# apache/cloudberry

Hardware: AMD Instinct MI355X
Metric: tpch_q3_rows_per_sec (higher is better)
Workload: dtype f64; 1 GPU; tpch_q3_sf100; lineitem_rows=599977225, parallelism=mpp1, lineitem_key_format=none, groups=12779481

## Files before the change

### cloudberry_amd/__init__.py

```python
import ctypes
import os

import numpy as np

_ROOT = os.path.dirname(os.path.dirname(os.path.abspath(__file__)))
_SO = os.path.join(_ROOT, "cloudberry_amd", "libgpuexec.so")

TPCH_CUSTOMER, TPCH_ORDERS, TPCH_LINEITEM = 0, 1, 2
TPCH_LINEITEM_NUMERIC = 3
TPCH_LINEITEM_RLEKEY = 4
TPCH_LINEITEM_Q1 = 5
CUTOFF_19950315 = -1753

_STATUS = {0: "GX_OK", 1: "GX_ERR_HIP", 2: "GX_ERR_RCCL", 3: "GX_ERR_INVALID",
           4: "GX_ERR_CHECKSUM", 5: "GX_ERR_OOM", 6: "GX_ERR_NOGPU", 7: "GX_ERR_STATE"}


class GxError(RuntimeError):
    def __init__(self, status, detail=""):
        self.status = status
        super().__init__(f"{_STATUS.get(status, status)}: {detail}")


class _Group(ctypes.Structure):
# ... 204 lines not shown
                                    ctypes.POINTER(ctypes.c_int64),
                                    ctypes.POINTER(_GbStats)]
    lib.gx_test_gb_partial.argtypes = [ctypes.c_void_p, ctypes.c_void_p,
                                       ctypes.c_int, ctypes.c_int, ctypes.c_int,
                                       ctypes.c_void_p, ctypes.c_void_p,
                                       ctypes.c_int64,
                                       ctypes.POINTER(ctypes.c_int64)]
    lib.gx_test_gb_combine.argtypes = [ctypes.c_void_p, ctypes.c_void_p,
                                       ctypes.c_int64,
                                       ctypes.POINTER(ctypes.POINTER(_KvGroup)),
                                       ctypes.POINTER(ctypes.c_int64)]
    lib.gx_partition_multi.argtypes = [ctypes.c_void_p, ctypes.c_void_p,
                                       ctypes.c_void_p, ctypes.c_void_p,
                                       ctypes.c_int32, ctypes.c_int64,
                                       ctypes.c_int32, ctypes.c_void_p]
    lib.gx_q3_prepare.argtypes = [ctypes.c_void_p] * 4 + [ctypes.c_int32,
                                  ctypes.POINTER(ctypes.c_void_p)]
    lib.gx_q3_prepare_desc.argtypes = [ctypes.c_void_p, ctypes.POINTER(_Q3Desc),
                                       ctypes.POINTER(ctypes.c_void_p)]
    lib.gx_q3_set_numeric.argtypes = [ctypes.c_void_p, ctypes.c_int]
    lib.gx_q3_run.argtypes = [ctypes.c_void_p]
    lib.gx_q3_stats_get.argtypes = [ctypes.c_void_p, ctypes.POINTER(_Stats)]
    lib.gx_q3_dim_mode.argtypes = [ctypes.c_void_p, ctypes.POINTER(ctypes.c_int)]
    lib.gx_q3_result.argtypes = [ctypes.c_void_p, ctypes.POINTER(ctypes.POINTER(_Group)),
                                 ctypes.POINTER(ctypes.c_int64)]
    lib.gx_q3_topn.argtypes = [ctypes.c_void_p, ctypes.c_int, ctypes.c_void_p,
                               ctypes.POINTER(ctypes.c_int64)]
    lib.gx_q3_free.argtypes = [ctypes.c_void_p]
    lib.gx_free.argtypes = [ctypes.c_void_p]
    lib.gx_test_motion1.argtypes = [ctypes.c_void_p, ctypes.c_void_p, ctypes.c_int32,
                                    ctypes.c_int, ctypes.c_void_p, ctypes.c_void_p,
                                    ctypes.c_int64, ctypes.POINTER(ctypes.c_int64)]
    lib.gx_test_qual.argtypes = [ctypes.c_void_p, ctypes.c_void_p, ctypes.c_void_p,
                                 ctypes.c_int64, ctypes.c_int, ctypes.c_void_p,
                                 ctypes.c_void_p, ctypes.c_int64,
                                 ctypes.POINTER(ctypes.c_int64)]
    lib.gx_test_q3_from_qual.argtypes = [ctypes.c_void_p, ctypes.c_void_p,
                                         ctypes.c_int64, ctypes.c_void_p,
                                         ctypes.c_int32,
                                         ctypes.POINTER(ctypes.POINTER(_Group)),
                                         ctypes.POINTER(ctypes.c_int64)]
    lib.gx_test_m1.argtypes = [ctypes.c_void_p, ctypes.c_void_p,
                               ctypes.POINTER(_Filter), ctypes.c_int,
                               ctypes.c_int, ctypes.c_void_p, ctypes.c_uint64,
                               ctypes.c_void_p, ctypes.c_void_p,
                               ctypes.c_int64, ctypes.POINTER(ctypes.c_int64)]
# ... 91 lines not shown
    rc = lib().gx_selftest_motion_layout(
        c.ctypes.data, n, seg, scnt.ctypes.data, soff.ctypes.data,
        rcnt.ctypes.data, roff.ctypes.data, 0, 0, 0, 1, 300, None)
    if rc != 0:
        raise ValueError(f"gx_selftest_motion_layout: bad arguments ({rc})")
    return scnt, soff, rcnt, roff


def motion_table_layout(qual, kmin, kmax, nsegs, tf_pct=300):
    lay = _TblLayout()
    rc = lib().gx_selftest_motion_layout(None, 0, 0, None, None, None, None,
                                         qual, kmin, kmax, nsegs, tf_pct,
                                         ctypes.byref(lay))
    if rc != 0:
        raise ValueError(f"gx_selftest_motion_layout: bad arguments ({rc})")
    return _layout_dict(lay)


def unmatched_bound(nrows, lmin, lmax):
    return int(lib().gx_selftest_unmatched_bound(
        int(nrows), int(lmin) & (2**64 - 1), int(lmax) & (2**64 - 1)))


def gb_lds_groups(naggs):
    return int(lib().gx_gb_lds_groups(naggs))


def gb_sort(keys, key_null):
    keys = np.ascontiguousarray(keys, np.int64)
    key_null = np.ascontiguousarray(key_null, np.uint8)
    assert keys.ndim == 2 and keys.shape == key_null.shape
    n, nkeys = keys.shape
    perm = np.zeros(n, np.int64)
    rc = lib().gx_selftest_gb_sort(keys.ctypes.data, key_null.ctypes.data, n,
                                   nkeys, perm.ctypes.data)
    if rc != 0:
        raise ValueError(f"gx_selftest_gb_sort: bad arguments ({rc})")
    return perm


def _gb_desc(table, keys, aggs, quals, max_groups):
    d = _GbDesc()
    d.t = None if table is None else table._t
    d.nkeys = len(keys)
    for i, c in enumerate(keys[:GB_MAX_KEYS]):
        d.key_cols[i] = c
# ... 598 lines not shown
            pass


class Q3:
    def __init__(self, ctx, q, tables=()):
        self.ctx = ctx
        self._q = q
        self._tables = tables

    def run(self):
        self.ctx._chk(self.ctx._lib.gx_q3_run(self._q))
        return self

    def stats(self):
        s = _Stats()
        self.ctx._chk(self.ctx._lib.gx_q3_stats_get(self._q, ctypes.byref(s)))
        return {f: getattr(s, f) for f, _ in s._fields_}

    def dim_mode(self):
        m = ctypes.c_int()
        self.ctx._chk(self.ctx._lib.gx_q3_dim_mode(self._q, ctypes.byref(m)))
        return m.value

    def result(self):
        gp = ctypes.POINTER(_Group)()
        n = ctypes.c_int64()
        self.ctx._chk(self.ctx._lib.gx_q3_result(self._q, ctypes.byref(gp),
                                                 ctypes.byref(n)))
        n = n.value
        res = {"l_orderkey": np.array([gp[i].l_orderkey for i in range(n)], np.int64),
               "o_orderdate": np.array([gp[i].o_orderdate for i in range(n)], np.int32),
               "o_shippriority": np.array([gp[i].o_shippriority for i in range(n)], np.int32),
               "revenue": np.array([gp[i].revenue for i in range(n)], np.float64),
               "revenue_num": np.array([gp[i].revenue_num for i in range(n)], np.int64),
               "nitems": np.array([gp[i].nitems for i in range(n)], np.int64),
               "key_is_null": np.array([gp[i].key_is_null for i in range(n)],
                                       np.bool_),
               "attrs_null": np.array([gp[i].attrs_null for i in range(n)],
                                      np.bool_)}
        self.ctx._lib.gx_free(gp)
        return res

    def topn(self, n=10):
        out = (_Group * n)()
        m = ctypes.c_int64()
        self.ctx._chk(self.ctx._lib.gx_q3_topn(self._q, n, out, ctypes.byref(m)))
# ... 24 lines not shown
```

### cloudberry_amd/csrc/gx_gpuexec.hip

```cpp
#include "gx_internal.h"
#include "../../include/gpuexec.h"

#include <hip/hip_runtime.h>
#include <rccl/rccl.h>
#include <zlib.h>

extern "C" size_t ZSTD_decompress(void *dst, size_t dstCap, const void *src,
                                  size_t srcSize);
extern "C" unsigned ZSTD_isError(size_t code);

#include <algorithm>
#include <chrono>
#include <cstdio>
#include <cstdlib>
#include <cstring>
#include <string>
#include <vector>
#include <map>
#include <utility>


static char g_global_err[512] = "";

struct gx_ctx {
// ... 660 lines not shown
    }
}


struct gx_slotmap {
    uint64_t mask;
    int64_t kmin;
    double scale;
    __host__ __device__ __forceinline__ uint64_t slot0(uint64_t k) const
    {
        if (scale < 0.0)
            return gx_hmix64(k) & mask;
        uint64_t s = (uint64_t) ((double) (int64_t) (k - (uint64_t) kmin) * scale);
        return s > mask ? mask : s;
    }
};

struct gx_dimbits {
    const unsigned long long *bits;
    uint64_t kmin;
    uint64_t range;
};

__device__ __forceinline__ void d_dimbits_set_wave(unsigned long long *bits,
                                                   uint64_t kmin, uint64_t range,
                                                   bool act, uint64_t k)
{
    uint64_t d = k - kmin;
    act = act && d < range;
    unsigned long long w = d >> 6;
    unsigned long long bit = 1ULL << (d & 63);
    int lane = (int) (threadIdx.x & 63);
    unsigned long long todo = __ballot(act);
    while (todo)
    {
        int lead = __ffsll((long long) todo) - 1;
        unsigned long long w0 = __shfl(w, lead, 64);
        bool same = ((todo >> lane) & 1ULL) && w == w0;
        unsigned long long grp = __ballot(same);
        unsigned long long v = same ? bit : 0ULL;
        if (grp & (grp - 1))
            for (int o = 32; o; o >>= 1)
                v |= __shfl_xor(v, o, 64);
        if (lane == lead)
            atomicOr(&bits[w0], v);
        todo &= ~grp;
    }
}

__device__ __forceinline__ unsigned long long d_bloom_mask_of(uint64_t h)
{
    int b1 = (int) ((h >> 32) & 63);
    int b2 = (int) ((h >> 38) & 63);
    return (1ULL << b1) | (1ULL << b2);
}

__device__ __forceinline__ void d_bloom_set(unsigned long long *bloom,
                                            uint64_t wmask, uint64_t k)
{
    uint64_t h = gx_hmix64(k);
    atomicOr(&bloom[h & wmask], d_bloom_mask_of(h));
}

__device__ __forceinline__ bool d_bloom_test(const unsigned long long *bloom,
                                             uint64_t wmask, uint64_t k)
{
    uint64_t h = gx_hmix64(k);
    unsigned long long m = d_bloom_mask_of(h);
    return (bloom[h & wmask] & m) == m;
}
// ... 508 lines not shown
        }
        bool in_set = d_dim_contains<BM>(cset, cmask, bloom, bwmask, bm, ck);
        if (in_set == ANTI) continue;
        if constexpr (BM)
            k = (uint64_t) gx_col_get_nt<int64_t>(ok_s, ok_m, i);
        else
            k = (uint64_t) gx_col_get<int64_t>(ok_s, ok_m, i);
        uint64_t slot = smap.slot0(k);
        while (true)
        {
            KT prev = atomicCAS(&tkey[slot], (KT) 0, (KT) k);
            if (prev == (KT) 0)
            {
                d_slot_claim(tattr, tagg, slot, od,
                             gx_col_get<int32_t>(op_s, op_m, i));
                break;
            }
            if (prev == (KT) k) break;
            slot = (slot + 1) & tmask;
        }
    }
}

template <typename KT, bool VM = false, bool OUTER = false>
__global__ void k_li_probe_agg_t(const uint8_t *lk_s, gx_colmeta lk_m,
                                 const uint8_t *pr_s, gx_colmeta pr_m,
                                 const uint8_t *di_s, gx_colmeta di_m,
                                 const uint8_t *sh_s, gx_colmeta sh_m,
                                 const uint8_t *vmap, int fop, int32_t flit,
                                 const KT *tkey,
                                 gx_aggslot *tagg,
                                 gx_slotmap smap,
                                 unsigned long long *hits,
                                 unsigned long long *ukey = nullptr,
                                 double *urev = nullptr,
                                 unsigned long long *ucnt = nullptr,
                                 uint64_t umask = 0)
{
    uint64_t tmask = smap.mask;
    unsigned long long local_hits = 0;
    auto umiss = [&](uint64_t k, int64_t i) {
        if constexpr (OUTER)
        {
            uint64_t slot = d_unmatched_claim(ukey, umask, k);
            double price = gx_col_get<double>(pr_s, pr_m, i);
            double disc = gx_col_get<double>(di_s, di_m, i);
            atomicAdd(&urev[slot], price * (1.0 - disc));
            atomicAdd(&ucnt[slot], 1ULL);
        }
        else
        {
            (void) k; (void) i;
        }
    };
    auto hit = [&](uint64_t slot, int64_t i) {
        double price = gx_col_get<double>(pr_s, pr_m, i);
        double disc = gx_col_get<double>(di_s, di_m, i);
        atomicAdd(&tagg[slot].sum, price * (1.0 - disc));
        atomicAdd(&tagg[slot].cnt, 1.0);
        local_hits++;
    };
    int64_t i = blockIdx.x * (int64_t) blockDim.x + threadIdx.x;
    int64_t stride = gridDim.x * (int64_t) blockDim.x;
    for (; i < lk_m.nrows; i += stride)
    {
        if constexpr (VM)
            if (gx_vm_hidden(vmap, i)) continue;
        if (!gx_cmp(fop, gx_col_get<int32_t>(sh_s, sh_m, i), flit)) continue;
        uint64_t k = (uint64_t) gx_col_get<int64_t>(lk_s, lk_m, i);
        uint64_t slot = smap.slot0(k);
        uint64_t r = d_table_find(tkey, tmask, slot, tkey[slot], k);
        if (r != ~0ULL) hit(r, i);
        else umiss(k, i);
    }
    gx_wave_count_add(hits, local_hits);
}

static constexpr int RLE_MAX_PHYS = 4096;

template <typename KT, bool VM = false>
__global__ void k_li_probe_agg_rle(const uint8_t *lk_s, const gx_blockref *dir,
                                   int64_t nblocks,
                                   const uint8_t *pr_s, gx_colmeta pr_m,
                                   const uint8_t *di_s, gx_colmeta di_m,
                                   const uint8_t *sh_s, gx_colmeta sh_m,
                                   const uint8_t *vmap, int fop, int32_t flit,
                                   const KT *tkey,
                                   gx_aggslot *tagg,
                                   gx_slotmap smap,
                                   unsigned long long *hits, int *err)
{
    __shared__ uint32_t s_starts[RLE_MAX_PHYS + 1];
    __shared__ uint32_t s_part[256];
    __shared__ uint32_t s_bytepop[RLE_MAX_PHYS / 8];
// ... 1349 lines not shown
    uint8_t *dvmap = nullptr;
};

struct gx_q3 {
    gx_ctx *ctx = nullptr;
    gx_table *cust = nullptr, *ord = nullptr, *li = nullptr;
    gx_q3_desc desc{};
    bool sized = false;
    void *cset = nullptr;
    int cset_width = 8;
    uint64_t cmask = 0;
    unsigned long long *bloom = nullptr;
    uint64_t bwmask = 0;
    unsigned long long *dbits = nullptr;
    uint64_t dim_kmin = 0, dim_range = 0;
    int dim_bitmap = 0;
    int dim_mode = 0;
    void *tkey = nullptr;
    int key_width = 8;
    gx_slotmap smap{};
    gx_attrpair *tattr = nullptr;
    gx_aggslot *tagg = nullptr;
    uint64_t tmask = 0;
    unsigned long long *dcount = nullptr, *dhits = nullptr, *dmin = nullptr;
    unsigned long long *m_hist = nullptr, *m_cur = nullptr;
    unsigned long long *m_bloom_all = nullptr;
    unsigned long long *m_cnts_mine = nullptr, *m_cnts_all = nullptr;
    gx_ord_row *m_send1 = nullptr, *m_recv1 = nullptr;
    gx_qual_row *m_send2 = nullptr, *m_recv2 = nullptr;
    uint64_t m_send1_cap = 0, m_recv1_cap = 0, m_send2_cap = 0, m_recv2_cap = 0;
    uint8_t *dtext = nullptr;
    uint8_t *dmask = nullptr;
    uint8_t *qvm_dim = nullptr, *qvm_mid = nullptr, *qvm_fact = nullptr;
    std::map<std::pair<const gx_table *, int>, gx_col> mat;
    std::vector<void *> mat_mem;
    int64_t *r_okey = nullptr;
    int32_t *r_odate = nullptr, *r_oprio = nullptr;
    double *r_rev = nullptr;
    int64_t *r_cnt = nullptr;
    uint8_t *r_flags = nullptr;
    unsigned long long *ukey = nullptr, *ucnt_u = nullptr;
    double *urev = nullptr;
    uint64_t umask = 0;
    int64_t u_cap = 0;
    int numeric = 0;
    int empty = 0;
// ... 2029 lines not shown
        lineitem->cols.size() != 4) return GX_ERR_INVALID;
    gx_q3_desc d{};
    d.dim = customer;
    d.dim_key_col = 0;
    d.dim_filter = {1, 2, 0};
    d.mid = orders;
    d.mid_key_col = 0;
    d.mid_fk_col = 1;
    d.mid_attr1_col = 2;
    d.mid_attr2_col = 3;
    d.mid_filter = {2, 0, cutoff};
    d.fact = lineitem;
    d.fact_key_col = 0;
    d.fact_a_col = 1;
    d.fact_b_col = 2;
    d.fact_filter = {3, 1, cutoff};
    return gx_q3_prepare_desc(ctx, &d, out);
}

static void q3_free_runstate(gx_q3 *q)
{
    auto fr = [](auto *&p) { if (p) { (void) hipFree(p); p = nullptr; } };
    fr(q->cset); fr(q->bloom); fr(q->dbits); fr(q->tkey); fr(q->tattr); fr(q->tagg);
    fr(q->r_okey); fr(q->r_odate); fr(q->r_oprio); fr(q->r_rev); fr(q->r_cnt);
    fr(q->r_flags);
    fr(q->ukey); fr(q->ucnt_u); fr(q->urev);
    fr(q->dcount); fr(q->dhits); fr(q->dmin);
    fr(q->m_hist); fr(q->m_cur); fr(q->m_cnts_mine); fr(q->m_cnts_all);
    fr(q->m_bloom_all);
    fr(q->m_send1); fr(q->m_recv1); fr(q->m_send2); fr(q->m_recv2);
    fr(q->dtext);
    fr(q->dmask);
    fr(q->qvm_dim); fr(q->qvm_mid); fr(q->qvm_fact);
    for (void *pm : q->mat_mem) (void) hipFree(pm);
    q->mat_mem.clear();
    q->mat.clear();
    q->m_send1_cap = q->m_recv1_cap = q->m_send2_cap = q->m_recv2_cap = 0;
    q->sized = false;
}

static gx_status hbm_budget_check(gx_ctx *ctx, uint64_t want, const char *what)
{
    size_t free_b = 0, total_b = 0;
    HIP_CHK(ctx, hipMemGetInfo(&free_b, &total_b));
    long mb = env_int("GX_HBM_BUDGET_MB", 0);
    uint64_t budget = mb > 0 ? (uint64_t) mb << 20
// ... 70 lines not shown
    if (bitmap)
        HIP_CHK(ctx, hipMemsetAsync(q->dbits, 0,
                                    (q->dim_range + 63) / 64 * 8, s));
    else
    {
        HIP_CHK(ctx, hipMemsetAsync(q->cset, 0, (q->cmask + 1) * q->cset_width, s));
        HIP_CHK(ctx, hipMemsetAsync(q->bloom, 0, (q->bwmask + 1) * 8, s));
    }
    dim_launch_build(s, ck, D.dim_text_len > 0 ? q->dmask : nullptr, cm,
                     D.dim_filter.op, D.dim_filter.literal, cvm,
                     q->cset, q->cset_width, q->cmask, q->bloom, q->bwmask,
                     bitmap ? q->dbits : nullptr, q->dim_kmin, q->dim_range);
    return GX_OK;
}

static uint64_t q3_unmatched_bound(int64_t nrows, uint64_t lmin, uint64_t lmax)
{
    if (nrows <= 0) return 1;
    uint64_t span = lmax - lmin + 1;
    if (lmax < lmin || span == 0) span = (uint64_t) nrows;
    return std::min<uint64_t>((uint64_t) nrows, span) + 1;
}

static gx_status q3_alloc_table(gx_q3 *q, uint64_t tslots, int64_t qual)
{
    gx_ctx *ctx = q->ctx;
    auto fr = [](auto *&p) { if (p) { (void) hipFree(p); p = nullptr; } };
    fr(q->tkey); fr(q->tattr); fr(q->tagg);
    fr(q->r_okey); fr(q->r_odate); fr(q->r_oprio); fr(q->r_rev); fr(q->r_cnt);
    fr(q->r_flags);
    HIP_CHK(ctx, hipMalloc(&q->tkey, tslots * q->key_width));
    HIP_CHK(ctx, hipMalloc(&q->tattr, tslots * sizeof(gx_attrpair)));
    HIP_CHK(ctx, hipMalloc(&q->tagg, tslots * sizeof(gx_aggslot)));
    q->rescap = std::max<int64_t>(qual + q->u_cap, 1);
    HIP_CHK(ctx, hipMalloc(&q->r_okey, q->rescap * 8));
    HIP_CHK(ctx, hipMalloc(&q->r_odate, q->rescap * 4));
    HIP_CHK(ctx, hipMalloc(&q->r_oprio, q->rescap * 4));
    HIP_CHK(ctx, hipMalloc(&q->r_rev, q->rescap * 8));
    HIP_CHK(ctx, hipMalloc(&q->r_cnt, q->rescap * 8));
    HIP_CHK(ctx, hipMalloc(&q->r_flags, q->rescap));
    q->tmask = tslots - 1;
    return GX_OK;
}

static gx_status q3_size_and_alloc(gx_q3 *q)
{
    gx_ctx *ctx = q->ctx;
    hipStream_t s = ctx->stream;
    const gx_q3_desc &D = q->desc;
    const gx_col &ckk = q3_col(q, q->cust, D.dim_key_col);
    const gx_col &cm = q3_col(q, q->cust, D.dim_filter.col);
    const gx_col &oc = q3_col(q, q->ord, D.mid_fk_col),
                 &od = q3_col(q, q->ord, D.mid_filter.col);
    const uint8_t *cvm = q->qvm_dim ? q->qvm_dim : q->cust->dvmap;
    const uint8_t *ovm = q->qvm_mid ? q->qvm_mid : q->ord->dvmap;

    HIP_CHK(ctx, hipMalloc(&q->dcount, 8));
    HIP_CHK(ctx, hipMalloc(&q->dhits, 8));
    HIP_CHK(ctx, hipMalloc(&q->dmin, 8));

    HIP_CHK(ctx, hipMemsetAsync(q->dcount, 0, 8, s));
    HIP_CHK(ctx, hipMemsetAsync(q->dhits, 0, 8, s));
    HIP_CHK(ctx, hipMemsetAsync(q->dmin, 0xFF, 8, s));
    dim_launch_count(s, ckk, D.dim_text_len > 0 ? q->dmask : nullptr, cm,
// ... 136 lines not shown
        };
        if (q->dim_bitmap)
            launch_ocount((const unsigned int *) nullptr, std::true_type{});
        else
            by_width(q->cset_width, (const void *) q->cset, [&](auto *cs) {
                launch_ocount(cs, std::false_type{});
            });
        unsigned long long nq = 0, kmax = 0, kmin = 0;
        HIP_CHK(ctx, hipMemcpyAsync(&nq, q->dcount, 8, hipMemcpyDeviceToHost, s));
        HIP_CHK(ctx, hipMemcpyAsync(&kmax, q->dhits, 8, hipMemcpyDeviceToHost, s));
        HIP_CHK(ctx, hipMemcpyAsync(&kmin, q->dmin, 8, hipMemcpyDeviceToHost, s));
        HIP_CHK(ctx, hipStreamSynchronize(s));
        qual = (int64_t) nq;
        if (qual > 0 && kmin == 0)
        {
            set_err(ctx, "mid join key 0 found among qualifying rows: 0 is "
                         "the empty-slot sentinel (gpuexec.h "
                         "gx_q3_prepare_desc)%s", "");
            return GX_ERR_INVALID;
        }
        q->key_width = (kmax < (1ULL << 32)) ? 4 : 8;
        int tf = env_int("GX_TABLE_FACTOR_PCT", 300);
        uint64_t tslots = (uint64_t) pow2_at_least(qual * tf / 100 + 1);
        {
            gx_status st = hbm_budget_check(
                ctx,
                tslots * (q->key_width + 4 + 4 + 8 + 8) +
                    (uint64_t) std::max<int64_t>(qual, 1) * (8 + 4 + 4 + 8 + 8),
                "join/agg table");
            if (st != GX_OK) return st;
        }
        q->smap.mask = tslots - 1;
        q->smap.kmin = (int64_t) kmin;
        q->smap.scale = -1.0;
        if (qual > 0 && kmax >= kmin)
        {
            double range = (double) (kmax - kmin) + 1.0;
            if ((double) qual >= range / 64.0)
                q->smap.scale = (double) tslots / range;
        }
        {
            gx_status st = q3_alloc_table(q, tslots, qual);
            if (st != GX_OK) return st;
        }
    }
    HIP_CHK(ctx, hipStreamSynchronize(s));
    q->sized = true;
    return GX_OK;
}


static inline bool m1_prefilter_on(int dim_join) { return dim_join == 0; }

static void m1_launch_hist(hipStream_t s, const gx_col &od, const gx_col &oc,
                           const uint8_t *vmap, int32_t fop, int32_t flit,
                           int nsegs, int dim_join,
                           const unsigned long long *bloom_all, uint64_t bwmask,
                           unsigned long long *dhist)
{
    if (!m1_prefilter_on(dim_join)) bloom_all = nullptr;
    hipLaunchKernelGGL(k_ord_m1_hist, dim3(GRID), dim3(TPB), 0, s,
                       od.dstream, od.m, oc.dstream, oc.m, vmap,
                       fop, flit, nsegs, bloom_all, bwmask, dhist);
}

// ... 93 lines not shown
                            const uint8_t *lvm, int32_t fop, int32_t flit,
                            int key_width, const void *tkey,
                            gx_aggslot *tagg, gx_slotmap smap,
                            unsigned long long *dhits, bool outer,
                            unsigned long long *ukey, double *urev,
                            unsigned long long *ucnt_u, uint64_t umask)
{
    by_width(key_width, tkey, [&](auto *keys) {
        by_flag(lvm != nullptr, [&](auto vm) {
            by_flag(outer, [&](auto ou) {
                hipLaunchKernelGGL((k_li_probe_agg_t<std::decay_t<decltype(*keys)>,
                                                     decltype(vm)::value,
                                                     decltype(ou)::value>),
                                   dim3(GRID), dim3(TPB), 0, s,
                                   lk.dstream, lk.m, lp.dstream, lp.m,
                                   ld.dstream, ld.m, ls.dstream, ls.m, lvm,
                                   fop, flit, keys, tagg, smap, dhits,
                                   ukey, urev, ucnt_u, umask);
            });
        });
    });
}

static gx_status q3_launch_extract(gx_ctx *ctx, hipStream_t s, int key_width,
                                   const void *tkey, const gx_attrpair *tattr,
                                   const gx_aggslot *tagg, uint64_t tslots,
                                   int numeric, int64_t *r_okey,
                                   int32_t *r_odate, int32_t *r_oprio,
                                   double *r_rev, int64_t *r_cnt,
                                   unsigned long long *dcount)
{
    uint64_t etiles = (tslots + GX_EXTRACT_TILE - 1) / GX_EXTRACT_TILE;
    if (etiles > 0x7FFFFFFFULL)
    {
        set_err(ctx, "join/agg table too large for the extract grid%s", "");
        return GX_ERR_INVALID;
    }
    by_width(key_width, tkey, [&](auto *keys) {
        hipLaunchKernelGGL(k_extract<std::decay_t<decltype(*keys)>>,
                           dim3((unsigned) etiles), dim3(TPB), 0, s,
                           keys, tattr, tagg, tslots, numeric,
                           r_okey, r_odate, r_oprio, r_rev, r_cnt, dcount);
    });
    return GX_OK;
}

extern "C" gx_status gx_q3_set_numeric(gx_q3 *q, int on)
{
    if (!q) return GX_ERR_INVALID;
    if (on && q3_col(q, q->li, q->desc.fact_key_col).format == 1)
    {
        set_err(q->ctx, "numeric mode is not supported with a fused RLE fact "
                        "key (numeric+RLE); bind the key plain%s", "");
        return GX_ERR_INVALID;
    }
    q->numeric = on ? 1 : 0;
    return GX_OK;
}

extern "C" gx_status gx_q3_dim_mode(gx_q3 *q, int *mode)
{
    if (!q || !mode) return GX_ERR_INVALID;
    if (!q->ran) return GX_ERR_STATE;
    *mode = q->dim_mode;
    return GX_OK;
}

struct q3_runcols {
    const gx_col &ok, &oc, &od, &op;
    const gx_col &lk, &lp, &ld, &ls;
    const uint8_t *ovm, *lvm;
};

static gx_status q3_orders_local(gx_q3 *q, const q3_runcols &C, bool use_bitmap)
{
    gx_ctx *ctx = q->ctx;
    hipStream_t s = ctx->stream;
    const gx_q3_desc &D = q->desc;
    const gx_col &ok = C.ok, &oc = C.oc, &od = C.od, &op = C.op;
    uint64_t tslots = q->tmask + 1;
    HIP_CHK(ctx, hipMemsetAsync(q->tkey, 0, tslots * q->key_width, s));
    if (D.fact_join == 1)
    {
        HIP_CHK(ctx, hipMemsetAsync(q->ukey, 0, (q->umask + 1) * 8, s));
        HIP_CHK(ctx, hipMemsetAsync(q->urev, 0, (q->umask + 1) * 8, s));
        HIP_CHK(ctx, hipMemsetAsync(q->ucnt_u, 0, (q->umask + 1) * 8, s));
    }
    gx_dimbits dbm = {q->dbits, q->dim_kmin, q->dim_range};
    auto launch_build = [&](auto *tk, auto *cs, auto bmode) {
        by_flag(C.ovm != nullptr, [&](auto vm) {
            by_flag(D.dim_join != 0, [&](auto anti) {
                hipLaunchKernelGGL((k_orders_build<std::decay_t<decltype(*tk)>,
                                                   std::decay_t<decltype(*cs)>,
                                                   decltype(vm)::value,
                                                   decltype(anti)::value,
                                                   decltype(bmode)::value>),
                                   dim3(ORDERS_GRID), dim3(TPB), 0, s,
                                   ok.dstream, ok.m, oc.dstream, oc.m, od.dstream, od.m,
                                   op.dstream, op.m, C.ovm, D.mid_filter.op,
                                   (int32_t) D.mid_filter.literal, cs, q->cmask,
                                   q->bloom, q->bwmask, dbm,
                                   tk, q->tattr, q->tagg, q->smap);
            });
        });
    };
    by_width(q->key_width, q->tkey, [&](auto *tk) {
        if (use_bitmap)
            launch_build(tk, (const unsigned int *) nullptr, std::true_type{});
        else
            by_width(q->cset_width, (const void *) q->cset, [&](auto *cs) {
                launch_build(tk, cs, std::false_type{});
            });
    });
    return GX_OK;
}

static gx_status q3_orders_motion(gx_q3 *q, const q3_runcols &C,
                                  hipEvent_t dim_done, int64_t *qual_out,
                                  double *ms_motion)
{
    gx_ctx *ctx = q->ctx;
    const gx_q3_desc &D = q->desc;
    const gx_col &ok = C.ok, &oc = C.oc, &od = C.od, &op = C.op;
    if (!ctx->comm) { set_err(ctx, "nsegs>1 but gx_comm_init not called%s", ""); return GX_ERR_STATE; }
    int n = ctx->nsegs;
    hipStream_t ms = ctx->stream2;
    evholder mev0, mev1;
    HIP_CHK(ctx, mev0.create()); HIP_CHK(ctx, mev1.create());
    HIP_CHK(ctx, hipEventRecord(mev0, ms));

    auto grow = [&](auto *&p, uint64_t &cap, uint64_t want) -> gx_status {
        if (want <= cap) return GX_OK;
        if (p) (void) hipFree(p);
        p = nullptr;
        cap = 0;
// ... 177 lines not shown
        HIP_CHK(ctx, hipMemsetAsync(q->dmin, 0, 8, s));
        by_width(q->key_width, (const void *) q->tkey, [&](auto *keys) {
            by_flag(C.lvm != nullptr, [&](auto vm) {
                by_flag(D.fact_join == 1, [&](auto outer) {
                    hipLaunchKernelGGL((k_li_probe_agg_num<std::decay_t<decltype(*keys)>,
                                                           decltype(vm)::value,
                                                           decltype(outer)::value>),
                                       dim3(GRID), dim3(TPB), 0, s,
                                       lk.dstream, lk.m, lp.dstream, lp.m, ld.dstream, ld.m,
                                       ls.dstream, ls.m, C.lvm, D.fact_filter.op,
                                       (int32_t) D.fact_filter.literal, keys,
                                       (gx_aggslot_num *) q->tagg, q->smap,
                                       dhits, (int *) q->dmin,
                                       q->ukey, (unsigned long long *) q->urev,
                                       q->ucnt_u, q->umask);
                });
            });
        });
        int herr = 0;
        HIP_CHK(ctx, hipMemcpyAsync(&herr, q->dmin, 4, hipMemcpyDeviceToHost, s));
        HIP_CHK(ctx, hipStreamSynchronize(s));
        if (herr) { set_err(ctx, "numeric overflow in aggregation%s", ""); return GX_ERR_INVALID; }
    }
    else
        q3_launch_probe(
            s, lk, lp, ld, ls, C.lvm, D.fact_filter.op,
            (int32_t) D.fact_filter.literal, q->key_width, q->tkey, q->tagg,
            q->smap, dhits, D.fact_join == 1, q->ukey, q->urev, q->ucnt_u,
            q->umask);
    return GX_OK;
}

static gx_status q3_extract(gx_q3 *q)
{
    gx_ctx *ctx = q->ctx;
    hipStream_t s = ctx->stream;
    unsigned long long *dcount = q->dcount;
    HIP_CHK(ctx, hipMemsetAsync(dcount, 0, 8, s));
    if (q->r_flags)
        HIP_CHK(ctx, hipMemsetAsync(q->r_flags, 0, q->rescap, s));
    const int egrid = 32768;
    {
        gx_status est = q3_launch_extract(ctx, s, q->key_width, q->tkey, q->tattr,
                                          q->tagg, q->tmask + 1, q->numeric,
                                          q->r_okey, q->r_odate, q->r_oprio,
                                          q->r_rev, q->r_cnt, dcount);
        if (est != GX_OK) return est;
    }
    if (q->desc.fact_join == 1)
        hipLaunchKernelGGL(k_extract_u, dim3(egrid), dim3(TPB), 0, s,
                           q->ukey, q->urev, q->ucnt_u, q->umask + 1,
                           q->r_okey, q->r_odate, q->r_oprio, q->r_rev,
                           q->r_cnt, q->r_flags, dcount, q->rescap);
    return GX_OK;
}

extern "C" gx_status gx_q3_run(gx_q3 *q)
{
    if (!q) return GX_ERR_INVALID;
    gx_ctx *ctx = q->ctx;
    hipStream_t s = ctx->stream;
    memset(&q->stats, 0, sizeof q->stats);
    if (!q->sized)
    {
        gx_status st = q3_size_and_alloc(q);
        if (st != GX_OK) return st;
    }
    if (q->empty)
    {
// ... 9 lines not shown
    for (auto &e : ev) HIP_CHK(ctx, e.create());

    const gx_q3_desc &D = q->desc;
    const q3_runcols C = {
        q3_col(q, q->ord, D.mid_key_col), q3_col(q, q->ord, D.mid_fk_col),
        q3_col(q, q->ord, D.mid_filter.col), q3_col(q, q->ord, D.mid_attr2_col),
        q3_col(q, q->li, D.fact_key_col), q3_col(q, q->li, D.fact_a_col),
        q3_col(q, q->li, D.fact_b_col), q3_col(q, q->li, D.fact_filter.col),
        q->qvm_mid ? q->qvm_mid : q->ord->dvmap,
        q->qvm_fact ? q->qvm_fact : (q->li ? q->li->dvmap : nullptr)};

    bool local_path = ctx->nsegs == 1 && env_int("GX_FORCE_MOTION", 0) == 0;
    bool use_bitmap = q->dim_bitmap && local_path;
    q->dim_mode = use_bitmap ? 1 : 0;
    HIP_CHK(ctx, hipEventRecord(ev[0], s));
    {
        gx_status st = q3_build_dim(q, use_bitmap);
        if (st != GX_OK) return st;
    }
    HIP_CHK(ctx, hipEventRecord(ev[1], s));

    int64_t qual = 0;
    double ms_motion = 0.0;
    if (local_path)
    {
        gx_status st = q3_orders_local(q, C, use_bitmap);
        if (st != GX_OK) return st;
        qual = q->rescap;
    }
    else
    {
        gx_status st = q3_orders_motion(q, C, ev[1], &qual, &ms_motion);
        if (st != GX_OK) return st;
    }
    q->qual_orders = qual;
    HIP_CHK(ctx, hipEventRecord(ev[2], s));

    {
        gx_status st = q3_probe_agg(q, C);
        if (st != GX_OK) return st;
    }
    HIP_CHK(ctx, hipEventRecord(ev[3], s));

    {
        gx_status st = q3_extract(q);
        if (st != GX_OK) return st;
    }
    HIP_CHK(ctx, hipEventRecord(ev[4], s));

// ... 1459 lines not shown
            return 1;
        static_assert(sizeof(unsigned long long) == sizeof(uint64_t), "u64");
        gx_mlayout L = m_exchange_layout((const unsigned long long *) cnts_all,
                                         n, seg);
        for (int i = 0; i < n; i++) { scnt[i] = L.scnt[i]; rcnt[i] = L.rcnt[i]; }
        for (int i = 0; i <= n; i++) { soff[i] = L.soff[i]; roff[i] = L.roff[i]; }
    }
    if (layout)
    {
        if (qual < 0 || nsegs < 1 || tf_pct < 0) return 1;
        test_fill_layout(layout,
                         m3_table_layout(qual, kmin, kmax, nsegs, tf_pct),
                         kmin, kmax);
    }
    return 0;
}

extern "C" uint64_t gx_selftest_unmatched_bound(int64_t nrows, uint64_t lmin,
                                                uint64_t lmax)
{
    return q3_unmatched_bound(nrows, lmin, lmax);
}

extern "C" int64_t gx_selftest_rle_block_class(const uint8_t *stream,
                                               int64_t nbytes, int32_t *cls,
                                               int64_t cap)
{
    if (!stream || nbytes < 0 || (cap > 0 && !cls)) return -1;
    std::vector<gx_blockref> dir;
    int64_t rows = 0;
    if (parse_block_dir(stream, nbytes, dir, &rows) != GX_OK) return -1;
    for (int64_t b = 0; b < (int64_t) dir.size() && b < cap; b++)
        cls[b] = dir[b].cls;
    return (int64_t) dir.size();
}

extern "C" int gx_selftest_rccl(int device)
{
    if (hipSetDevice(device) != hipSuccess) return 1;
    ncclUniqueId id;
    if (ncclGetUniqueId(&id) != ncclSuccess) return 2;
    ncclComm_t comm;
    if (ncclCommInitRank(&comm, 1, id, 0) != ncclSuccess) return 3;
    devbuf a, b;
    if (a.alloc(8) != hipSuccess || b.alloc(8) != hipSuccess) return 4;
    unsigned long long v = 0xC0FFEE;
// ... 38 lines not shown
```

### include/gpuexec.h

```cpp
#ifndef GPUEXEC_H
#define GPUEXEC_H

#include <stdint.h>
#include <stddef.h>

#ifdef __cplusplus
extern "C" {
#endif

typedef enum gx_status {
    GX_OK = 0,
    GX_ERR_HIP = 1,
    GX_ERR_RCCL = 2,
    GX_ERR_INVALID = 3,
    GX_ERR_CHECKSUM = 4,
    GX_ERR_OOM = 5,
    GX_ERR_NOGPU = 6,
    GX_ERR_STATE = 7
} gx_status;

typedef struct gx_ctx gx_ctx;
typedef struct gx_table gx_table;
typedef struct gx_q3 gx_q3;

// ... 115 lines not shown
    int32_t mid_attr2_col;
    gx_filter mid_filter;
    gx_table *fact;
    int32_t fact_key_col;
    int32_t fact_a_col;
    int32_t fact_b_col;
    gx_filter fact_filter;
    char dim_text[64];
    int32_t dim_text_len;
#define GX_MAX_EXTRA_QUALS 4
    gx_filter dim_extra[GX_MAX_EXTRA_QUALS];
    gx_filter mid_extra[GX_MAX_EXTRA_QUALS];
    gx_filter fact_extra[GX_MAX_EXTRA_QUALS];
    int32_t n_dim_extra, n_mid_extra, n_fact_extra;
    int32_t dim_join;
    int32_t fact_join;
} gx_q3_desc;

gx_status gx_q3_prepare_desc(gx_ctx *ctx, const gx_q3_desc *desc, gx_q3 **out);
gx_status gx_q3_set_numeric(gx_q3 *q, int on);
gx_status gx_q3_run(gx_q3 *q);
gx_status gx_q3_stats_get(const gx_q3 *q, gx_q3_stats *out);
gx_status gx_q3_dim_mode(gx_q3 *q, int *mode);
gx_status gx_q3_result(gx_q3 *q, gx_q3_group **out, int64_t *ngroups);
gx_status gx_q3_topn(gx_q3 *q, int topn, gx_q3_group *out, int64_t *nout);
gx_status gx_q3_free(gx_q3 *q);

void gx_free(void *p);

int64_t gx_abi_sizeof(int kind);

typedef struct gx_kv_group {
    int64_t key;
    uint8_t key_is_null;
    uint8_t _pad[7];
    double  sum;
    int64_t count;
} gx_kv_group;
gx_status gx_groupby(gx_ctx *ctx, const gx_table *t, int key_col, int val_col,
                     gx_kv_group **out, int64_t *ngroups);

typedef struct gx_gb_stats {
    double  ms_partial, ms_partition, ms_exchange, ms_combine;
    int64_t rows_in, partial_groups, sent_rows, recv_rows, final_groups;
} gx_gb_stats;

// ... 85 lines not shown
gx_status gx_test_m3(gx_ctx *ctx, const gx_qual_row_abi *rows, int64_t n,
                     gx_table *lineitem, int32_t op, int64_t literal,
                     gx_q3_group **out, int64_t *ngroups,
                     gx_test_tbl_layout *layout);
int gx_selftest_motion_layout(const uint64_t *cnts_all, int n, int seg,
                              uint64_t *scnt, uint64_t *soff,
                              uint64_t *rcnt, uint64_t *roff,
                              int64_t qual, uint64_t kmin, uint64_t kmax,
                              int nsegs, int tf_pct,
                              gx_test_tbl_layout *layout);


gx_status gx_test_topn(gx_ctx *ctx, const int64_t *okey, const int32_t *odate,
                       const int32_t *oprio, const double *rev,
                       const int64_t *cnt, const uint8_t *flags, int64_t n,
                       int numeric, int topn, gx_q3_group *out, int64_t *nout);
int gx_selftest_topn_merge(const int64_t *cidx, const int64_t *okey,
                           const int32_t *odate, const int32_t *oprio,
                           const double *rev, const int64_t *cnt,
                           const uint8_t *flags, int ncand, int numeric,
                           int topn, gx_q3_group *out, int64_t *nout);
uint64_t gx_selftest_unmatched_bound(int64_t nrows, uint64_t lmin,
                                     uint64_t lmax);
int64_t gx_selftest_rle_block_class(const uint8_t *stream, int64_t nbytes,
                                    int32_t *cls, int64_t cap);

#ifdef __cplusplus
}
#endif
#endif
```

Baseline: 87.20 billion rows/s.

## Replace Q3 hash join table with dense rank-bitmap table for compact key ranges

Adds a rank-table path for the local Q3 join/aggregate. When the qualifying order-key span is under 64 times the qualifying count, orders are marked in a bitmap and a prefix-popcount scan assigns dense indices. A fill kernel then writes keys and attributes into dense arrays, and the lineitem probe uses a single bitmap lookup with popcount instead of hash probing. This is meant to remove hash-probe cost and shrink table memory. It adds extra orders-side passes (mark, three scan kernels, fill) and only applies to non-numeric, uncompressed-key local runs.

```diff
diff --git a/cloudberry_amd/__init__.py b/cloudberry_amd/__init__.py
--- a/cloudberry_amd/__init__.py
+++ b/cloudberry_amd/__init__.py
@@ -250,6 +250,12 @@
     lib.gx_q3_run.argtypes = [ctypes.c_void_p]
     lib.gx_q3_stats_get.argtypes = [ctypes.c_void_p, ctypes.POINTER(_Stats)]
     lib.gx_q3_dim_mode.argtypes = [ctypes.c_void_p, ctypes.POINTER(ctypes.c_int)]
+    lib.gx_q3_table_mode.argtypes = [ctypes.c_void_p, ctypes.POINTER(ctypes.c_int)]
+    lib.gx_selftest_rank_eligible.restype = ctypes.c_int
+    lib.gx_selftest_rank_eligible.argtypes = [ctypes.c_int64, ctypes.c_uint64,
+                                              ctypes.c_uint64, ctypes.c_int]
+    lib.gx_rank_scan_block_keys.restype = ctypes.c_int64
+    lib.gx_rank_scan_block_keys.argtypes = []
     lib.gx_q3_result.argtypes = [ctypes.c_void_p, ctypes.POINTER(ctypes.POINTER(_Group)),
                                  ctypes.POINTER(ctypes.c_int64)]
     lib.gx_q3_topn.argtypes = [ctypes.c_void_p, ctypes.c_int, ctypes.c_void_p,
@@ -387,6 +393,16 @@
         int(nrows), int(lmin) & (2**64 - 1), int(lmax) & (2**64 - 1)))
 
 
+def rank_eligible(qual, kmin, kmax, enabled=True):
+    return bool(lib().gx_selftest_rank_eligible(
+        int(qual), int(kmin) & (2**64 - 1), int(kmax) & (2**64 - 1),
+        1 if enabled else 0))
+
+
+def rank_scan_block_keys():
+    return int(lib().gx_rank_scan_block_keys())
+
+
 def gb_lds_groups(naggs):
     return int(lib().gx_gb_lds_groups(naggs))
 
@@ -1031,6 +1047,15 @@
         self.ctx._chk(self.ctx._lib.gx_q3_dim_mode(self._q, ctypes.byref(m)))
         return m.value
 
+    def set_numeric(self, on=True):
+        self.ctx._chk(self.ctx._lib.gx_q3_set_numeric(self._q, 1 if on else 0))
+        return self
+
+    def table_mode(self):
+        m = ctypes.c_int()
+        self.ctx._chk(self.ctx._lib.gx_q3_table_mode(self._q, ctypes.byref(m)))
+        return m.value
+
     def result(self):
         gp = ctypes.POINTER(_Group)()
         n = ctypes.c_int64()
diff --git a/cloudberry_amd/csrc/gx_gpuexec.hip b/cloudberry_amd/csrc/gx_gpuexec.hip
--- a/cloudberry_amd/csrc/gx_gpuexec.hip
+++ b/cloudberry_amd/csrc/gx_gpuexec.hip
@@ -706,6 +706,7 @@
     uint64_t range;
 };
 
+template <int STRIDE = 1>
 __device__ __forceinline__ void d_dimbits_set_wave(unsigned long long *bits,
                                                    uint64_t kmin, uint64_t range,
                                                    bool act, uint64_t k)
@@ -727,9 +728,26 @@
             for (int o = 32; o; o >>= 1)
                 v |= __shfl_xor(v, o, 64);
         if (lane == lead)
-            atomicOr(&bits[w0], v);
+            atomicOr(&bits[w0 * STRIDE], v);
         todo &= ~grp;
     }
+}
+
+struct gx_rankview {
+    const ulonglong2 *ent;
+    uint64_t kmin, range, qual;
+};
+
+static constexpr int GX_RANK_SCAN_WORDS = 8 * TPB;
+
+__device__ __forceinline__ uint64_t d_rank_find(const gx_rankview &rv, uint64_t k)
+{
+    uint64_t d = k - rv.kmin;
+    if (d >= rv.range) return ~0ULL;
+    ulonglong2 e = rv.ent[d >> 6];
+    int sh = (int) (d & 63);
+    uint64_t idx = e.y + (uint64_t) __popcll(e.x & ((1ULL << sh) - 1ULL));
+    return (((e.x >> sh) & 1ULL) && idx < rv.qual) ? idx : ~0ULL;
 }
 
 __device__ __forceinline__ unsigned long long d_bloom_mask_of(uint64_t h)
@@ -1284,7 +1302,130 @@
     }
 }
 
-template <typename KT, bool VM = false, bool OUTER = false>
+
+template <typename KS, bool VM = false, bool ANTI = false, bool BM = false>
+__global__ void k_orders_mark(const uint8_t *ok_s, gx_colmeta ok_m,
+                              const uint8_t *oc_s, gx_colmeta oc_m,
+                              const uint8_t *od_s, gx_colmeta od_m,
+                              const uint8_t *vmap, int oop, int32_t olit,
+                              const KS *cset, uint64_t cmask,
+                              const unsigned long long *bloom, uint64_t bwmask,
+                              gx_dimbits bm,
+                              ulonglong2 *rent, uint64_t kmin,
+                              uint64_t range, unsigned long long *rowmask)
+{
+    const int lane = (int) (threadIdx.x & 63);
+    int64_t base = blockIdx.x * (int64_t) blockDim.x + threadIdx.x - lane;
+    int64_t stride = gridDim.x * (int64_t) blockDim.x;
+    for (; base < ok_m.nrows; base += stride)
+    {
+        int64_t r = base + lane;
+        bool act = r < ok_m.nrows;
+        if constexpr (VM)
+            act = act && !gx_vm_hidden(vmap, r);
+        uint64_t ck = 0, k = 0;
+        if constexpr (BM)
+        {
+            int32_t od = 0;
+            if (act)
+            {
+                od = gx_col_get_nt<int32_t>(od_s, od_m, r);
+                ck = (uint64_t) gx_col_get_nt<int64_t>(oc_s, oc_m, r);
+            }
+            act = act && gx_cmp(oop, od, olit);
+        }
+        else
+        {
+            act = act && gx_cmp(oop, gx_col_get<int32_t>(od_s, od_m, r), olit);
+            if (act) ck = (uint64_t) gx_col_get<int64_t>(oc_s, oc_m, r);
+        }
+        if (act)
+            act = d_dim_contains<BM>(cset, cmask, bloom, bwmask, bm, ck) != ANTI;
+        if (act)
+        {
+            if constexpr (BM)
+                k = (uint64_t) gx_col_get_nt<int64_t>(ok_s, ok_m, r);
+            else
+                k = (uint64_t) gx_col_get<int64_t>(ok_s, ok_m, r);
+        }
+        act = act && (k - kmin) < range;
+        d_dimbits_set_wave<2>(reinterpret_cast<unsigned long long *>(rent),
+                              kmin, range, act, k);
+        unsigned long long m = __ballot(act);
+        if (lane == 0) rowmask[base >> 6] = m;
+    }
+}
+
+__global__ void __launch_bounds__(TPB)
+k_rank_blocksum(const ulonglong2 *rent, uint64_t nwords, uint32_t *blk)
+{
+    __shared__ uint32_t s_w[TPB / 64];
+    uint64_t w0 = (uint64_t) blockIdx.x * GX_RANK_SCAN_WORDS;
+    uint32_t acc = 0;
+    for (int j = threadIdx.x; j < GX_RANK_SCAN_WORDS; j += TPB)
+    {
+        uint64_t w = w0 + (uint64_t) j;
+        if (w < nwords)
+            acc += (uint32_t) __popcll(rent[w].x);
+    }
+    for (int o = 32; o; o >>= 1)
+        acc += __shfl_down(acc, o, 64);
+    if ((threadIdx.x & 63) == 0) s_w[threadIdx.x >> 6] = acc;
+    __syncthreads();
+    if (threadIdx.x == 0)
+    {
+        uint32_t t = 0;
+        for (int i = 0; i < TPB / 64; i++) t += s_w[i];
+        blk[blockIdx.x] = t;
+    }
+}
+
+__global__ void __launch_bounds__(TPB)
+k_rank_topscan(uint32_t *blk, int nblk)
+{
+    __shared__ uint32_t s_part[TPB];
+    d_block_excl_scan(blk, nblk, s_part, nullptr, [&](int i) { return blk[i]; });
+}
+
+__global__ void __launch_bounds__(TPB)
+k_rank_localscan(ulonglong2 *rent, uint64_t nwords, const uint32_t *blk)
+{
+    __shared__ uint32_t s_scan[GX_RANK_SCAN_WORDS];
+    __shared__ uint32_t s_part[TPB];
+    uint64_t w0 = (uint64_t) blockIdx.x * GX_RANK_SCAN_WORDS;
+    int n = (nwords - w0 < (uint64_t) GX_RANK_SCAN_WORDS)
+                ? (int) (nwords - w0) : GX_RANK_SCAN_WORDS;
+    d_block_excl_scan(s_scan, n, s_part, nullptr, [&](int i) {
+        return (uint32_t) __popcll(rent[w0 + (uint64_t) i].x);
+    });
+    uint32_t b0 = blk[blockIdx.x];
+    for (int j = threadIdx.x; j < n; j += TPB)
+        rent[w0 + (uint64_t) j].y = (unsigned long long) (b0 + s_scan[j]);
+}
+
+template <typename KT>
+__global__ void k_orders_fill(const uint8_t *ok_s, gx_colmeta ok_m,
+                              const uint8_t *od_s, gx_colmeta od_m,
+                              const uint8_t *op_s, gx_colmeta op_m,
+                              const unsigned long long *rowmask, gx_rankview rv,
+                              KT *dkey, gx_attrpair *dattr, gx_aggslot *dagg)
+{
+    int64_t i = blockIdx.x * (int64_t) blockDim.x + threadIdx.x;
+    int64_t stride = gridDim.x * (int64_t) blockDim.x;
+    for (; i < ok_m.nrows; i += stride)
+    {
+        if (!((rowmask[i >> 6] >> (i & 63)) & 1ULL)) continue;
+        uint64_t k = (uint64_t) gx_col_get<int64_t>(ok_s, ok_m, i);
+        int32_t a1 = gx_col_get<int32_t>(od_s, od_m, i);
+        int32_t a2 = gx_col_get<int32_t>(op_s, op_m, i);
+        uint64_t idx = d_rank_find(rv, k);
+        if (idx == ~0ULL) continue;
+        dkey[idx] = (KT) k;
+        d_slot_claim(dattr, dagg, idx, a1, a2);
+    }
+}
+
+template <typename KT, bool VM = false, bool OUTER = false, bool RANK = false>
 __global__ void k_li_probe_agg_t(const uint8_t *lk_s, gx_colmeta lk_m,
                                  const uint8_t *pr_s, gx_colmeta pr_m,
                                  const uint8_t *di_s, gx_colmeta di_m,
@@ -1297,7 +1438,8 @@
                                  unsigned long long *ukey = nullptr,
                                  double *urev = nullptr,
                                  unsigned long long *ucnt = nullptr,
-                                 uint64_t umask = 0)
+                                 uint64_t umask = 0,
+                                 gx_rankview rv = {})
 {
     uint64_t tmask = smap.mask;
     unsigned long long local_hits = 0;
@@ -1330,8 +1472,14 @@
             if (gx_vm_hidden(vmap, i)) continue;
         if (!gx_cmp(fop, gx_col_get<int32_t>(sh_s, sh_m, i), flit)) continue;
         uint64_t k = (uint64_t) gx_col_get<int64_t>(lk_s, lk_m, i);
-        uint64_t slot = smap.slot0(k);
-        uint64_t r = d_table_find(tkey, tmask, slot, tkey[slot], k);
+        uint64_t r;
+        if constexpr (RANK)
+            r = d_rank_find(rv, k);
+        else
+        {
+            uint64_t slot = smap.slot0(k);
+            r = d_table_find(tkey, tmask, slot, tkey[slot], k);
+        }
         if (r != ~0ULL) hit(r, i);
         else umiss(k, i);
     }
@@ -2727,6 +2875,17 @@
     gx_attrpair *tattr = nullptr;
     gx_aggslot *tagg = nullptr;
     uint64_t tmask = 0;
+    uint64_t hash_tslots = 0;
+    int64_t local_qual = 0;
+    int rank_ok = 0, rank_kw = 8;
+    int table_mode = 0;
+    uint64_t rank_kmin = 0, rank_range = 0;
+    ulonglong2 *rent = nullptr;
+    uint32_t *rblk = nullptr;
+    unsigned long long *rowmask = nullptr;
+    void *dkey = nullptr;
+    gx_attrpair *dattr = nullptr;
+    gx_aggslot *dagg = nullptr;
     unsigned long long *dcount = nullptr, *dhits = nullptr, *dmin = nullptr;
     unsigned long long *m_hist = nullptr, *m_cur = nullptr;
     unsigned long long *m_bloom_all = nullptr;
@@ -4802,6 +4961,8 @@
 {
     auto fr = [](auto *&p) { if (p) { (void) hipFree(p); p = nullptr; } };
     fr(q->cset); fr(q->bloom); fr(q->dbits); fr(q->tkey); fr(q->tattr); fr(q->tagg);
+    fr(q->rent); fr(q->rblk); fr(q->rowmask);
+    fr(q->dkey); fr(q->dattr); fr(q->dagg);
     fr(q->r_okey); fr(q->r_odate); fr(q->r_oprio); fr(q->r_rev); fr(q->r_cnt);
     fr(q->r_flags);
     fr(q->ukey); fr(q->ucnt_u); fr(q->urev);
@@ -4918,24 +5079,79 @@
     return std::min<uint64_t>((uint64_t) nrows, span) + 1;
 }
 
+static gx_status q3_alloc_results(gx_q3 *q, int64_t qual);
+static gx_status q3_alloc_hash(gx_q3 *q, uint64_t tslots);
+
 static gx_status q3_alloc_table(gx_q3 *q, uint64_t tslots, int64_t qual)
+{
+    gx_status st = q3_alloc_hash(q, tslots);
+    if (st != GX_OK) return st;
+    return q3_alloc_results(q, qual);
+}
+
+static gx_status q3_alloc_results(gx_q3 *q, int64_t qual)
 {
     gx_ctx *ctx = q->ctx;
     auto fr = [](auto *&p) { if (p) { (void) hipFree(p); p = nullptr; } };
-    fr(q->tkey); fr(q->tattr); fr(q->tagg);
     fr(q->r_okey); fr(q->r_odate); fr(q->r_oprio); fr(q->r_rev); fr(q->r_cnt);
     fr(q->r_flags);
-    HIP_CHK(ctx, hipMalloc(&q->tkey, tslots * q->key_width));
-    HIP_CHK(ctx, hipMalloc(&q->tattr, tslots * sizeof(gx_attrpair)));
-    HIP_CHK(ctx, hipMalloc(&q->tagg, tslots * sizeof(gx_aggslot)));
-    q->rescap = std::max<int64_t>(qual + q->u_cap, 1);
+    q->rescap = std::max<int64_t>(std::max(qual, q->local_qual) + q->u_cap, 1);
     HIP_CHK(ctx, hipMalloc(&q->r_okey, q->rescap * 8));
     HIP_CHK(ctx, hipMalloc(&q->r_odate, q->rescap * 4));
     HIP_CHK(ctx, hipMalloc(&q->r_oprio, q->rescap * 4));
     HIP_CHK(ctx, hipMalloc(&q->r_rev, q->rescap * 8));
     HIP_CHK(ctx, hipMalloc(&q->r_cnt, q->rescap * 8));
     HIP_CHK(ctx, hipMalloc(&q->r_flags, q->rescap));
+    return GX_OK;
+}
+
+static gx_status q3_alloc_hash(gx_q3 *q, uint64_t tslots)
+{
+    gx_ctx *ctx = q->ctx;
+    auto fr = [](auto *&p) { if (p) { (void) hipFree(p); p = nullptr; } };
+    fr(q->tkey); fr(q->tattr); fr(q->tagg);
+    gx_status st = hbm_budget_check(
+        ctx, tslots * (q->key_width + sizeof(gx_attrpair) + sizeof(gx_aggslot)),
+        "join/agg table");
+    if (st != GX_OK) return st;
+    HIP_CHK(ctx, hipMalloc(&q->tkey, tslots * q->key_width));
+    HIP_CHK(ctx, hipMalloc(&q->tattr, tslots * sizeof(gx_attrpair)));
+    HIP_CHK(ctx, hipMalloc(&q->tagg, tslots * sizeof(gx_aggslot)));
     q->tmask = tslots - 1;
+    return GX_OK;
+}
+
+static bool q3_rank_eligible(int64_t qual, uint64_t kmin, uint64_t kmax,
+                             int enabled)
+{
+    if (!enabled || qual <= 0 || kmax < kmin) return false;
+    if ((uint64_t) qual >= (1ULL << 32)) return false;
+    uint64_t span = kmax - kmin;
+    return span < 64 * (uint64_t) qual;
+}
+
+static gx_status q3_alloc_rank(gx_q3 *q)
+{
+    gx_ctx *ctx = q->ctx;
+    uint64_t nwords = (q->rank_range + 63) / 64;
+    uint64_t nblk = (nwords + GX_RANK_SCAN_WORDS - 1) / GX_RANK_SCAN_WORDS;
+    uint64_t qual = (uint64_t) q->local_qual;
+    uint64_t mwords = ((uint64_t) q->ord->nrows + 63) / 64;
+    auto fr = [](auto *&p) { if (p) { (void) hipFree(p); p = nullptr; } };
+    fr(q->rent); fr(q->rblk); fr(q->rowmask);
+    fr(q->dkey); fr(q->dattr); fr(q->dagg);
+    gx_status st = hbm_budget_check(
+        ctx,
+        nwords * 16 + nblk * 4 + mwords * 8 +
+            qual * (q->rank_kw + sizeof(gx_attrpair) + sizeof(gx_aggslot)),
+        "rank join/agg table");
+    if (st != GX_OK) return st;
+    HIP_CHK(ctx, hipMalloc(&q->rent, nwords * sizeof(ulonglong2)));
+    HIP_CHK(ctx, hipMalloc(&q->rblk, nblk * 4));
+    HIP_CHK(ctx, hipMalloc(&q->rowmask, std::max<uint64_t>(mwords, 1) * 8));
+    HIP_CHK(ctx, hipMalloc(&q->dkey, qual * q->rank_kw));
+    HIP_CHK(ctx, hipMalloc(&q->dattr, qual * sizeof(gx_attrpair)));
+    HIP_CHK(ctx, hipMalloc(&q->dagg, qual * sizeof(gx_aggslot)));
     return GX_OK;
 }
 
@@ -5118,6 +5334,13 @@
         q->key_width = (kmax < (1ULL << 32)) ? 4 : 8;
         int tf = env_int("GX_TABLE_FACTOR_PCT", 300);
         uint64_t tslots = (uint64_t) pow2_at_least(qual * tf / 100 + 1);
+        q->rank_ok = q3_rank_eligible(qual, kmin, kmax,
+                                      env_int("GX_RANK_TABLE", 1) != 0);
+        q->rank_kmin = q->rank_ok ? kmin : 0;
+        q->rank_range = q->rank_ok ? kmax - kmin + 1 : 0;
+        q->rank_kw = q->key_width;
+        q->local_qual = qual;
+        q->hash_tslots = tslots;
         {
             gx_status st = hbm_budget_check(
                 ctx,
@@ -5136,7 +5359,7 @@
                 q->smap.scale = (double) tslots / range;
         }
         {
-            gx_status st = q3_alloc_table(q, tslots, qual);
+            gx_status st = q3_alloc_results(q, qual);
             if (st != GX_OK) return st;
         }
     }
@@ -5276,6 +5499,29 @@
     });
 }
 
+static void q3_launch_probe_rank(hipStream_t s,
+                                 const gx_col &lk, const gx_col &lp,
+                                 const gx_col &ld, const gx_col &ls,
+                                 const uint8_t *lvm, int32_t fop, int32_t flit,
+                                 gx_rankview rv, gx_aggslot *dagg,
+                                 unsigned long long *dhits, bool outer,
+                                 unsigned long long *ukey, double *urev,
+                                 unsigned long long *ucnt_u, uint64_t umask)
+{
+    by_flag(lvm != nullptr, [&](auto vm) {
+        by_flag(outer, [&](auto ou) {
+            hipLaunchKernelGGL((k_li_probe_agg_t<uint32_t, decltype(vm)::value,
+                                                 decltype(ou)::value, true>),
+                               dim3(GRID), dim3(TPB), 0, s,
+                               lk.dstream, lk.m, lp.dstream, lp.m,
+                               ld.dstream, ld.m, ls.dstream, ls.m, lvm,
+                               fop, flit, (const uint32_t *) nullptr, dagg,
+                               gx_slotmap{}, dhits,
+                               ukey, urev, ucnt_u, umask, rv);
+        });
+    });
+}
+
 static gx_status q3_launch_extract(gx_ctx *ctx, hipStream_t s, int key_width,
                                    const void *tkey, const gx_attrpair *tattr,
                                    const gx_aggslot *tagg, uint64_t tslots,
@@ -5320,6 +5566,14 @@
     return GX_OK;
 }
 
+extern "C" gx_status gx_q3_table_mode(gx_q3 *q, int *mode)
+{
+    if (!q || !mode) return GX_ERR_INVALID;
+    if (!q->ran) return GX_ERR_STATE;
+    *mode = q->table_mode;
+    return GX_OK;
+}
+
 struct q3_runcols {
     const gx_col &ok, &oc, &od, &op;
     const gx_col &lk, &lp, &ld, &ls;
@@ -5332,6 +5586,11 @@
     hipStream_t s = ctx->stream;
     const gx_q3_desc &D = q->desc;
     const gx_col &ok = C.ok, &oc = C.oc, &od = C.od, &op = C.op;
+    if (q->tkey == nullptr)
+    {
+        gx_status st = q3_alloc_hash(q, q->hash_tslots);
+        if (st != GX_OK) return st;
+    }
     uint64_t tslots = q->tmask + 1;
     HIP_CHK(ctx, hipMemsetAsync(q->tkey, 0, tslots * q->key_width, s));
     if (D.fact_join == 1)
@@ -5365,6 +5624,79 @@
             by_width(q->cset_width, (const void *) q->cset, [&](auto *cs) {
                 launch_build(tk, cs, std::false_type{});
             });
+    });
+    return GX_OK;
+}
+
+static inline gx_rankview q3_rankview(const gx_q3 *q)
+{
+    return {q->rent, q->rank_kmin, q->rank_range, (uint64_t) q->local_qual};
+}
+
+static gx_status q3_orders_rank(gx_q3 *q, const q3_runcols &C, bool use_bitmap)
+{
+    gx_ctx *ctx = q->ctx;
+    hipStream_t s = ctx->stream;
+    const gx_q3_desc &D = q->desc;
+    const gx_col &ok = C.ok, &oc = C.oc, &od = C.od, &op = C.op;
+    if (q->dagg == nullptr)
+    {
+        gx_status st = q3_alloc_rank(q);
+        if (st != GX_OK) return st;
+    }
+    uint64_t nwords = (q->rank_range + 63) / 64;
+    uint64_t nblk = (nwords + GX_RANK_SCAN_WORDS - 1) / GX_RANK_SCAN_WORDS;
+    if (nblk > 0x7FFFFFFFULL)
+    {
+        set_err(ctx, "rank table too large for the scan grid%s", "");
+        return GX_ERR_INVALID;
+    }
+    HIP_CHK(ctx, hipMemsetAsync(q->rent, 0, nwords * sizeof(ulonglong2), s));
+    HIP_CHK(ctx, hipMemsetAsync(q->dkey, 0,
+                                (uint64_t) q->local_qual * q->rank_kw, s));
+    if (D.fact_join == 1)
+    {
+        HIP_CHK(ctx, hipMemsetAsync(q->ukey, 0, (q->umask + 1) * 8, s));
+        HIP_CHK(ctx, hipMemsetAsync(q->urev, 0, (q->umask + 1) * 8, s));
+        HIP_CHK(ctx, hipMemsetAsync(q->ucnt_u, 0, (q->umask + 1) * 8, s));
+    }
+    gx_dimbits dbm = {q->dbits, q->dim_kmin, q->dim_range};
+    const gx_rankview rv = q3_rankview(q);
+    auto launch_mark = [&](auto *cs, auto bmode) {
+        by_flag(C.ovm != nullptr, [&](auto vm) {
+            by_flag(D.dim_join != 0, [&](auto anti) {
+                hipLaunchKernelGGL((k_orders_mark<std::decay_t<decltype(*cs)>,
+                                                  decltype(vm)::value,
+                                                  decltype(anti)::value,
+                                                  decltype(bmode)::value>),
+                                   dim3(ORDERS_GRID), dim3(TPB), 0, s,
+                                   ok.dstream, ok.m, oc.dstream, oc.m,
+                                   od.dstream, od.m, C.ovm, D.mid_filter.op,
+                                   (int32_t) D.mid_filter.literal, cs, q->cmask,
+                                   q->bloom, q->bwmask, dbm,
+                                   q->rent, q->rank_kmin, q->rank_range,
+                                   q->rowmask);
+            });
+        });
+    };
+    if (use_bitmap)
+        launch_mark((const unsigned int *) nullptr, std::true_type{});
+    else
+        by_width(q->cset_width, (const void *) q->cset, [&](auto *cs) {
+            launch_mark(cs, std::false_type{});
+        });
+    hipLaunchKernelGGL(k_rank_blocksum, dim3((unsigned) nblk), dim3(TPB), 0, s,
+                       q->rent, nwords, q->rblk);
+    hipLaunchKernelGGL(k_rank_topscan, dim3(1), dim3(TPB), 0, s,
+                       q->rblk, (int) nblk);
+    hipLaunchKernelGGL(k_rank_localscan, dim3((unsigned) nblk), dim3(TPB), 0, s,
+                       q->rent, nwords, q->rblk);
+    by_width(q->rank_kw, q->dkey, [&](auto *dk) {
+        hipLaunchKernelGGL(k_orders_fill<std::decay_t<decltype(*dk)>>,
+                           dim3(ORDERS_GRID), dim3(TPB), 0, s,
+                           ok.dstream, ok.m, od.dstream, od.m,
+                           op.dstream, op.m, q->rowmask, rv, dk,
+                           q->dattr, q->dagg);
     });
     return GX_OK;
 }
@@ -5588,6 +5920,12 @@
         HIP_CHK(ctx, hipStreamSynchronize(s));
         if (herr) { set_err(ctx, "numeric overflow in aggregation%s", ""); return GX_ERR_INVALID; }
     }
+    else if (q->table_mode == 1)
+        q3_launch_probe_rank(
+            s, lk, lp, ld, ls, C.lvm, D.fact_filter.op,
+            (int32_t) D.fact_filter.literal, q3_rankview(q),
+            q->dagg, dhits, D.fact_join == 1, q->ukey, q->urev, q->ucnt_u,
+            q->umask);
     else
         q3_launch_probe(
             s, lk, lp, ld, ls, C.lvm, D.fact_filter.op,
@@ -5607,10 +5945,15 @@
         HIP_CHK(ctx, hipMemsetAsync(q->r_flags, 0, q->rescap, s));
     const int egrid = 32768;
     {
-        gx_status est = q3_launch_extract(ctx, s, q->key_width, q->tkey, q->tattr,
-                                          q->tagg, q->tmask + 1, q->numeric,
-                                          q->r_okey, q->r_odate, q->r_oprio,
-                                          q->r_rev, q->r_cnt, dcount);
+        gx_status est = q->table_mode == 1
+            ? q3_launch_extract(ctx, s, q->rank_kw, q->dkey, q->dattr, q->dagg,
+                                (uint64_t) q->local_qual, q->numeric,
+                                q->r_okey, q->r_odate, q->r_oprio,
+                                q->r_rev, q->r_cnt, dcount)
+            : q3_launch_extract(ctx, s, q->key_width, q->tkey, q->tattr,
+                                q->tagg, q->tmask + 1, q->numeric,
+                                q->r_okey, q->r_odate, q->r_oprio,
+                                q->r_rev, q->r_cnt, dcount);
         if (est != GX_OK) return est;
     }
     if (q->desc.fact_join == 1)
@@ -5666,9 +6009,12 @@
 
     int64_t qual = 0;
     double ms_motion = 0.0;
+    q->table_mode = (q->rank_ok && local_path && !q->numeric &&
+                     C.lk.format == 0) ? 1 : 0;
     if (local_path)
     {
-        gx_status st = q3_orders_local(q, C, use_bitmap);
+        gx_status st = q->table_mode == 1 ? q3_orders_rank(q, C, use_bitmap)
+                                          : q3_orders_local(q, C, use_bitmap);
         if (st != GX_OK) return st;
         qual = q->rescap;
     }
@@ -7174,6 +7520,17 @@
     return q3_unmatched_bound(nrows, lmin, lmax);
 }
 
+extern "C" int gx_selftest_rank_eligible(int64_t qual, uint64_t kmin,
+                                         uint64_t kmax, int enabled)
+{
+    return q3_rank_eligible(qual, kmin, kmax, enabled) ? 1 : 0;
+}
+
+extern "C" int64_t gx_rank_scan_block_keys(void)
+{
+    return (int64_t) GX_RANK_SCAN_WORDS * 64;
+}
+
 extern "C" int64_t gx_selftest_rle_block_class(const uint8_t *stream,
                                                int64_t nbytes, int32_t *cls,
                                                int64_t cap)
diff --git a/include/gpuexec.h b/include/gpuexec.h
--- a/include/gpuexec.h
+++ b/include/gpuexec.h
@@ -161,6 +161,7 @@
 gx_status gx_q3_run(gx_q3 *q);
 gx_status gx_q3_stats_get(const gx_q3 *q, gx_q3_stats *out);
 gx_status gx_q3_dim_mode(gx_q3 *q, int *mode);
+gx_status gx_q3_table_mode(gx_q3 *q, int *mode);
 gx_status gx_q3_result(gx_q3 *q, gx_q3_group **out, int64_t *ngroups);
 gx_status gx_q3_topn(gx_q3 *q, int topn, gx_q3_group *out, int64_t *nout);
 gx_status gx_q3_free(gx_q3 *q);
@@ -292,6 +293,9 @@
                            int topn, gx_q3_group *out, int64_t *nout);
 uint64_t gx_selftest_unmatched_bound(int64_t nrows, uint64_t lmin,
                                      uint64_t lmax);
+int gx_selftest_rank_eligible(int64_t qual, uint64_t kmin, uint64_t kmax,
+                              int enabled);
+int64_t gx_rank_scan_block_keys(void);
 int64_t gx_selftest_rle_block_class(const uint8_t *stream, int64_t nbytes,
                                     int32_t *cls, int64_t cap);
 
```

New measurement: 97.98 billion rows/s, median of 6. +12.4%, better.
